# tomerlieber/doc-agents

Hardware: AMD Instinct MI355X
Metric: QA queries/sec + p50 cache-miss latency; docs/min ingest at 1/2/4/8 MI355X (higher is better)
Workload: dtype bf16

## Files before the change

### docagents_amd/models/llama.py

```python
from __future__ import annotations

import numpy as np
import torch

from ..ops import get_ops
from ..ops.reference import interleave_gate_up, rope_table
from .configs import DecoderConfig

EPI_NONE, EPI_SWIGLU, EPI_RESID, EPI_ROPE = 0, 3, 4, 6
_FUSED_ROPE_DECODE = True


class TPContext:

    def __init__(self, rank: int = 0, size: int = 1, group=None, xgmi: bool = True):
        self.rank, self.size, self.group = rank, size, group
        self.use_xgmi = xgmi
        self.xgmi = None
        self.xgmi_norm = None

    def setup_device(self, device: torch.device) -> None:
        if self.size > 1 and device.type == "cuda" and self.xgmi is None and self.use_xgmi:
            from ..parallel.xgmi_allreduce import XgmiAllReduce
            self.xgmi = XgmiAllReduce.create(self.group, device)
            if self.xgmi is not None:
                self.xgmi_norm = XgmiAllReduce.create(self.group, device, max_bytes=512 << 10)

    def close(self) -> None:
        comms = [c for c in (self.xgmi, self.xgmi_norm) if c is not None]
        if not comms:
            return
        import torch.distributed as dist
        dist.barrier(group=self.group)
# ... 202 lines not shown
    def _attn_out_and_mlp(self, L, a, x):
        o, tp = self.ops, self.tp
        if tp.size == 1 or tp.rank == 0:
            self._gemm1(L, "wo", a, epi=EPI_RESID, resid=x, out=x)
        else:
            o.gemm(a, L["wo"], out=x)
        tp.all_reduce_(x)
        return self._mlp(L, x)

    def _mlp(self, L, x):
        o, tp = self.ops, self.tp
        if o.gemv_fusable(x.shape[0], L["w_gu"].shape[0], x.shape[1], EPI_SWIGLU):
            g = self._gemm1(L, "w_gu", x, epi=EPI_SWIGLU, rms=(self._gain(L["ln_mlp"]), self.cfg.eps))
        else:
            h = o.rmsnorm(x, L["ln_mlp"], self.cfg.eps)
            g = o.gemm(h, L["w_gu"], epi=EPI_SWIGLU)
        if tp.size == 1 or tp.rank == 0:
            self._gemm1(L, "w_down", g, epi=EPI_RESID, resid=x, out=x)
        else:
            o.gemm(g, L["w_down"], out=x)
        tp.all_reduce_(x)
        return x

    def _logits(self, hlast, gather: bool = True, out=None):
        o = self.ops
        if o.gemv_fusable(hlast.shape[0], self.w["lm_head"].shape[0], hlast.shape[1]):
            logits = self._gemm1(self.w, "lm_head", hlast.contiguous(), rms=(self._gain(self.w["norm"]), self.cfg.eps),
                                 out=None if gather else out)
        else:
            h = o.rmsnorm(hlast, self.w["norm"], self.cfg.eps)
            logits = o.gemm(h, self.w["lm_head"], out=None if gather else out)
        return self.tp.all_gather_cols(logits) if gather else logits

    def sample(self, logits, temperature: float, seed: int, step: int = 0, **kw):
        return tp_sample(self.ops, self.tp, logits, temperature, seed, step, **kw)

    def prefill(self, ids: torch.Tensor, pos: torch.Tensor, slot_tok: torch.Tensor, cu: torch.Tensor,
                max_seqlen: int, last_idx: torch.Tensor, prefix: tuple[int, int] | None = None,
                local_logits: bool = False) -> torch.Tensor:
        c, o, cache = self.cfg, self.ops, self.cache
        D, hl, kl = c.head_dim, self.hl, self.kl
        x = o.embed(ids, self.w["embed"])
        hook = self.layer_hook
        kv_from_cache = bool(getattr(o, "flash_kv_cache_ok", lambda *_: False)(D, True))
        for li, L in enumerate(self.w["layers"]):
            if hook is not None:
                hook(li)
            h = o.rmsnorm(x, L["ln_attn"], c.eps)
            qkv = o.gemm_rope(h, L["wqkv"], pos, self.cos_sin, hl, kl, D, slot_tok, cache.k(li), cache.v(li),
                              kv_out=not kv_from_cache)
            pre = None if prefix is None else (cache.k(li)[prefix[0]], cache.v(li)[prefix[0]], prefix[1])
            if kv_from_cache:
                a = o.flash_attn_varlen(qkv[:, :hl * D], None, None, cu, max_seqlen, hl, kl, D, causal=True,
                                        prefix=pre, kv_cache=(cache.k(li), cache.v(li), slot_tok, pos))
            else:
                a = o.flash_attn_varlen(qkv[:, :hl * D], qkv[:, hl * D:(hl + kl) * D], qkv[:, (hl + kl) * D:], cu,
                                        max_seqlen, hl, kl, D, causal=True, prefix=pre)
            del qkv, h
            x = self._attn_out_and_mlp(L, a, x)
        return self._logits(x.index_select(0, last_idx), gather=not local_logits)

    def decode_step(self, st: "DecodeState") -> torch.Tensor:
        c, o, cache = self.cfg, self.ops, self.cache
        D, hl, kl = c.head_dim, self.hl, self.kl
        x = o.embed(st.tokens, self.w["embed"], out=st.x)
        if self._dk_decode(x.shape[0]):
            return self._decode_step_dk(st, x)
        if self._norm_fusable(x.shape[0]):
            return self._decode_step_fused_norms(st, x)
        if self.tp.size > 1 and x.shape[0] > 1:
            return self._decode_step_tp_fused_norms(st, x)
        fuse = o.gemv_fusable(x.shape[0], self.w["layers"][0]["wqkv"].shape[0], x.shape[1])
        for li, L in enumerate(self.w["layers"]):
            if fuse:
                qkv = self._gemm1(L, "wqkv", x, out=st.qkv, rms=(self._gain(L["ln_attn"]), c.eps))
            else:
                h = o.rmsnorm(x, L["ln_attn"], c.eps, out=st.h)
                qkv = o.gemm(h, L["wqkv"], out=st.qkv)
            a = self._decode_attn(qkv, li, st)
            self._attn_out_and_mlp(L, a, x)
        logits = self._logits(x, gather=False, out=st.logits)
# ... 140 lines not shown
```

### docagents_amd/ops/csrc/attention.hip

```cpp
#include "common.h"

#include <cstdlib>

#pragma clang fp contract(on)

template <int D, int NW = 4, int QH = 1>
struct FA2Cfg {
  static constexpr int KT = 64, QW = 32 * QH, QB = QW * NW, NT = 64 * NW;
  static constexpr int KSTR = D * 2 + 16;
  static constexpr int VSTR = (D == 64) ? 192 : (D == 128) ? 320 : D * 2;
  static constexpr int KBUF = KT * KSTR, VBUF = KT * VSTR;
  static constexpr int CPR = D / 8, LPT = (KT * CPR + NT - 1) / NT;
  static constexpr int SMEM = 2 * (KBUF + VBUF);
};

struct FaPrefix {
  const bf16_t* k;
  const bf16_t* v;
  long long hstride;
  int len;
  int rev;
  const int* kv_slot;
  const int* kv_pos;
  const bf16_t* kc;
  const bf16_t* vc;
  long long slot_stride;
};

struct FaBlock {
  int qb, h, b;
};
__device__ __forceinline__ FaBlock fa_block(int rev, int causal, int G) {
  const int X = gridDim.x, Y = gridDim.y, Z = gridDim.z;
  const bool lpt = causal && (rev & 1);
  if ((rev & 2) && G >= 1 && Y % G == 0 && ((Y / G) * Z) % 8 == 0) {
    const int g = blockIdx.x + X * (blockIdx.y + Y * blockIdx.z);
    const int xcd = g & 7, s = g >> 3;
    const int per = X * G;
    const int pair = (s / per) * 8 + xcd, r = s % per;
    const int qi = r / G, gh = r % G;
    const int hkv = Y / G;
    return FaBlock{lpt ? X - 1 - qi : qi, (pair % hkv) * G + gh, pair / hkv};
  }
  return FaBlock{lpt ? X - 1 - (int)blockIdx.x : (int)blockIdx.x, (int)blockIdx.y, (int)blockIdx.z};
}

template <int D, int NW, int QH, typename T = BF16T>
__global__ void __launch_bounds__(64 * NW, QH == 1 ? 8 / NW : 1)
flash_attn_v2_kernel(const bf16_t* __restrict__ q, const bf16_t* __restrict__ k, const bf16_t* __restrict__ v,
                     int ldq, int ldk, int ldv, const int* __restrict__ cu, int H, int Hkv, int causal,
                     float c, bf16_t* __restrict__ o, int ldo, FaPrefix pre) {
  using C = FA2Cfg<D, NW, QH>;
  constexpr int KT = C::KT, NDS = D / 16, NDB = D / 32, CPR = C::CPR, LPT = C::LPT, NT = C::NT;
  constexpr bool EVEN = (KT * CPR) % NT == 0;
  extern __shared__ __attribute__((aligned(16))) char smem[];

  const FaBlock fb = fa_block(pre.rev, causal, H / Hkv);
  const int b = fb.b, h = fb.h, qb = fb.qb;
  const int s0 = cu[b], L = cu[b + 1] - s0;
  const int q0 = qb * C::QB;
  if (q0 >= L) return;
  const int hk = h / (H / Hkv);
  const int tid = threadIdx.x, lane = tid & 63, wid = tid >> 6;
  const int qr = lane & 31, hi = lane >> 5;
  const int wq0 = q0 + wid * C::QW;
  int qi[QH];
  bool qvalid[QH];
  bf16x8_t qf[QH][NDS];
  f32x16_t oacc[QH][NDB];
  float m_run[QH], l_part[QH];
#pragma unroll
  for (int j = 0; j < QH; ++j) {
    qi[j] = wq0 + 32 * j + qr;
    qvalid[j] = qi[j] < L;
#pragma unroll
    for (int ds = 0; ds < NDS; ++ds) {
      if (qvalid[j]) qf[j][ds] = *(const bf16x8_t*)(q + (size_t)(s0 + qi[j]) * ldq + h * D + ds * 16 + hi * 8);
      else qf[j][ds] = bf16x8_t{0, 0, 0, 0, 0, 0, 0, 0};
    }
#pragma unroll
    for (int i = 0; i < NDB; ++i)
#pragma unroll
// ... 221 lines not shown
      "s_add_u32 m0, m0, 0x400\n\t"
      "s_nop 0\n\t"
      "buffer_load_dwordx4 %3, %4, %6 offen lds\n\t"
      "s_mov_b32 m0, %0"
      : "=&s"(keep)
      : "v"(v0), "v"(v1), "v"(v2), "s"(rs), "s"(lds), "s"(soff)
      : "memory", "scc");
}

template <int D, bool SPEC, bool DMA>
__global__ void __launch_bounds__(256, 2)
flash_attn_pipe_kernel(const bf16_t* __restrict__ q, const bf16_t* __restrict__ k, const bf16_t* __restrict__ v,
                       int ldq, int ldk, int ldv, const int* __restrict__ cu, int H, int Hkv, int causal,
                       float c, bf16_t* __restrict__ o, int ldo, FaPrefix pre) {
  using C = FA2Cfg<D, 4, 1>;
  constexpr int KT = C::KT, NDS = D / 16, NDB = D / 32, CPR = C::CPR, LPT = C::LPT, NT = C::NT;
  constexpr bool EVEN = (KT * CPR) % NT == 0;
  static_assert(NDS <= 6, "pipelined flash: D <= 96");
  static_assert(!DMA || (D == 96 && C::VSTR == D * 2), "DMA tiles: D = 96 (linear V rows)");
  constexpr int KSTR = DMA ? D * 2 : C::KSTR, KBUF = KT * KSTR, TBUF = KBUF + C::VBUF;
  extern __shared__ __attribute__((aligned(16))) char smem[];

  const FaBlock fb = fa_block(pre.rev, causal, H / Hkv);
  const int b = fb.b, h = fb.h, qb = fb.qb;
  const int s0 = cu[b], L = cu[b + 1] - s0;
  const int q0 = qb * C::QB;
  if (q0 >= L) return;
  const int hk = h / (H / Hkv);
  const int tid = threadIdx.x, lane = tid & 63, wid = tid >> 6;
  const int qr = lane & 31, hi = lane >> 5;
  const int wq0 = q0 + wid * C::QW;
  const int qi = wq0 + qr;
  const bool qvalid = qi < L;
  bf16x8_t qf[NDS];
#pragma unroll
  for (int ds = 0; ds < NDS; ++ds)
    qf[ds] = qvalid ? *(const bf16x8_t*)(q + (size_t)(s0 + qi) * ldq + h * D + ds * 16 + hi * 8)
                    : bf16x8_t{0, 0, 0, 0, 0, 0, 0, 0};
  f32x16_t oacc[NDB];
#pragma unroll
  for (int i = 0; i < NDB; ++i)
#pragma unroll
    for (int r = 0; r < 16; ++r) oacc[i][r] = 0.f;
  float m_run = -INFINITY, l_part = 0.f;

  const int P = pre.len, Lk = P + L;
  const int kv_end = causal ? min(Lk, P + q0 + C::QB) : Lk;
  const int wave_end = causal ? min(Lk, P + wq0 + C::QW) : Lk;
// ... 1207 lines not shown
#define FA_ARGS16 (const bf16_t*)q, (const bf16_t*)k, (const bf16_t*)v, ldq, ldk, ldv, (const int*)cu_seqlens, H, Hkv, \
                  causal, scale * 1.4426950408889634f, (bf16_t*)o, ldo, pre
  switch (D) {
    case 64: flash_attn_v2_kernel<64, 4, 1, F16T><<<grid, 256, FA2Cfg<64, 4, 1>::SMEM, s>>>(FA_ARGS16); break;
    case 96: flash_attn_v2_kernel<96, 4, 1, F16T><<<grid, 256, FA2Cfg<96, 4, 1>::SMEM, s>>>(FA_ARGS16); break;
    default: return (int)hipErrorInvalidValue;
  }
#undef FA_ARGS16
  return (int)hipGetLastError();
}

template <int NW, int QH>
static int launch_fa2(const void* q, const void* k, const void* v, int ldq, int ldk, int ldv, const void* cu_seqlens,
                      int B, int max_seqlen, int H, int Hkv, int D, int causal, float sl2e, void* o, int ldo,
                      FaPrefix pre, hipStream_t s) {
  static bool attr_set = false;
  if constexpr (NW * QH <= 8) {
    if (!attr_set) {
      (void)hipFuncSetAttribute((const void*)flash_attn_v2_kernel<128, NW, QH>, hipFuncAttributeMaxDynamicSharedMemorySize,
                                FA2Cfg<128, NW, QH>::SMEM);
      attr_set = true;
    }
  }
  dim3 grid((max_seqlen + 32 * QH * NW - 1) / (32 * QH * NW), H, B);
#define FA_ARGS (const bf16_t*)q, (const bf16_t*)k, (const bf16_t*)v, ldq, ldk, ldv, (const int*)cu_seqlens, H, Hkv, \
                causal, sl2e, (bf16_t*)o, ldo, pre
  switch (D) {
    case 32: flash_attn_v2_kernel<32, NW, QH><<<grid, 64 * NW, FA2Cfg<32, NW, QH>::SMEM, s>>>(FA_ARGS); break;
    case 64: flash_attn_v2_kernel<64, NW, QH><<<grid, 64 * NW, FA2Cfg<64, NW, QH>::SMEM, s>>>(FA_ARGS); break;
    case 96:
      if constexpr (NW * QH <= 8) flash_attn_v2_kernel<96, NW, QH><<<grid, 64 * NW, FA2Cfg<96, NW, QH>::SMEM, s>>>(FA_ARGS);
      else return (int)hipErrorInvalidValue;
      break;
    case 128:
      if constexpr (NW * QH <= 8) flash_attn_v2_kernel<128, NW, QH><<<grid, 64 * NW, FA2Cfg<128, NW, QH>::SMEM, s>>>(FA_ARGS);
      else return (int)hipErrorInvalidValue;
      break;
    default: return (int)hipErrorInvalidValue;
  }
#undef FA_ARGS
  return (int)hipGetLastError();
}

template <int D, bool DMA>
static constexpr int fa_pipe_smem() {
  return 3 * ((DMA ? 64 * D * 2 : FA2Cfg<D, 4, 1>::KBUF) + FA2Cfg<D, 4, 1>::VBUF);
}

template <bool DMA>
static int launch_fa_pipe(const void* q, const void* k, const void* v, int ldq, int ldk, int ldv, const void* cu_seqlens,
                          int B, int max_seqlen, int H, int Hkv, int causal, float sl2e, void* o, int ldo,
                          FaPrefix pre, hipStream_t s) {
  static bool attr_set = false;
  if (!attr_set) {
    (void)hipFuncSetAttribute((const void*)flash_attn_pipe_kernel<96, true, DMA>,
                              hipFuncAttributeMaxDynamicSharedMemorySize, fa_pipe_smem<96, DMA>());
    attr_set = true;
  }
  dim3 grid((max_seqlen + 127) / 128, H, B);
  flash_attn_pipe_kernel<96, true, DMA><<<grid, 256, fa_pipe_smem<96, DMA>(), s>>>(
      (const bf16_t*)q, (const bf16_t*)k, (const bf16_t*)v, ldq, ldk, ldv, (const int*)cu_seqlens, H, Hkv, causal, sl2e,
      (bf16_t*)o, ldo, pre);
  return (int)hipGetLastError();
}

DA_EXPORT int da_flash_attn_v2(const void* q, const void* k, const void* v, int ldq, int ldk, int ldv,
                               const void* cu_seqlens, int B, int max_seqlen, int H, int Hkv, int D, int causal,
                               float scale, void* o, int ldo, const void* pre_k, const void* pre_v,
                               long long pre_hstride, int pre_len, const void* kv_slot, const void* kv_pos,
                               const void* k_cache, const void* v_cache, void* stream) {
  const bool from_cache = kv_slot != nullptr;
  if (from_cache) {
    if (!causal || D != 96 || !kv_pos || !k_cache || !v_cache || pre_hstride < (long long)D ||
        pre_hstride % D || ((uintptr_t)k_cache | (uintptr_t)v_cache) % 16)
      return (int)hipErrorInvalidValue;
    k = k_cache; v = v_cache; ldk = ldv = D;
  }
  if (H % Hkv || ldq % 8 || ldk % 8 || ldv % 8 || ldo % 4) return (int)hipErrorInvalidValue;
  if (pre_len < 0 || (pre_len > 0 && (!pre_k || !pre_v || pre_hstride < (long long)pre_len * D)))
    return (int)hipErrorInvalidValue;
  if (B == 0 || max_seqlen == 0) return 0;
  const float sl2e = scale * 1.4426950408889634f;
  hipStream_t s = (hipStream_t)stream;
  const FaPrefix pre{(const bf16_t*)pre_k, (const bf16_t*)pre_v, pre_hstride, pre_len, kFaDispatch,
                     (const int*)kv_slot, (const int*)kv_pos, (const bf16_t*)k_cache, (const bf16_t*)v_cache,
                     from_cache ? (long long)Hkv * pre_hstride : 0LL};
  if (causal && D == 96) {
    const bool dma = pre_len % 64 == 0 && ((uintptr_t)k | (uintptr_t)v | (uintptr_t)pre_k | (uintptr_t)pre_v) % 16 == 0;
    if (dma) return launch_fa_pipe<true>(q, k, v, ldq, ldk, ldv, cu_seqlens, B, max_seqlen, H, Hkv, causal, sl2e, o, ldo, pre, s);
    return launch_fa_pipe<false>(q, k, v, ldq, ldk, ldv, cu_seqlens, B, max_seqlen, H, Hkv, causal, sl2e, o, ldo, pre, s);
  }
  if (D == 128) return launch_fa2<8, 1>(q, k, v, ldq, ldk, ldv, cu_seqlens, B, max_seqlen, H, Hkv, D, causal, sl2e, o, ldo, pre, s);
  return launch_fa2<4, 1>(q, k, v, ldq, ldk, ldv, cu_seqlens, B, max_seqlen, H, Hkv, D, causal, sl2e, o, ldo, pre, s);
}
```

### docagents_amd/ops/csrc/gemm.hip

```cpp
#include "gemm.h"

template <int BM, int BN, int WM, int WN, int EPI, int PF = 1>
__global__ void __launch_bounds__(256)
gemm_bf16_kernel(GemmArgs p) {
  constexpr int BK = 64;
  constexpr int TM = BM / WM, TN = BN / WN;
  constexpr int FM = TM / 16, FN = TN / 16;
  constexpr int A_BYTES = BM * BK * 2, B_BYTES = BN * BK * 2;
  constexpr int LA = BM * 8 / 256, LB = BN * 8 / 256;
  static_assert(WM * WN == 4, "4 waves");
  static_assert(LA >= 1 && LB >= 1, "tile too small");
  constexpr int STAGE_FLOATS = 4 * TM * (TN + 4);
  constexpr int LDS_MAIN = 2 * (A_BYTES + B_BYTES);
  constexpr int LDS_BYTES = LDS_MAIN > STAGE_FLOATS * 4 ? LDS_MAIN : STAGE_FLOATS * 4;
  __shared__ __attribute__((aligned(16))) char smem[LDS_BYTES];

  const int tid = threadIdx.x, lane = tid & 63, wid = tid >> 6;
  const int wm = wid / WN, wn = wid % WN;

  const int ntm = (p.M + BM - 1) / BM, ntn = (p.N + BN - 1) / BN;
  const int nwg = ntm * ntn;
  const int t = xcd_remap(blockIdx.x, nwg);
  constexpr int GROUP = 8;
  const int gid = t / (GROUP * ntn);
// ... 507 lines not shown
  const int nout = (epi == EPI_SWIGLU) ? N / 2 : N;
  const size_t work = (size_t)M * (nout / 8);
  const int blocks = (int)((work + 255) / 256);
  gemm_splitk_reduce<<<blocks, 256, 0, s>>>((const float*)ws, splits, M, N, epi, (const bf16_t*)bias,
                                             (const bf16_t*)resid, ldr, (bf16_t*)C, ldc, ssq_in, ssq_parts, norm_k,
                                             eps);
  DA_LAUNCH_CHECK();
}

DA_EXPORT int da_gemm_rope(const void* A, int lda, const void* W, void* C, int ldc, int M, int N, int K,
                           const void* pos, const void* slot, const void* cos_sin, void* k_cache, void* v_cache,
                           int H, int Hkv, int D, int max_seq, int kv_out, void* stream) {
  if (K % 64 || K < 128 || N % 8 || lda % 8 || ldc % 8 || D % 8 || M < 256) return (int)hipErrorInvalidValue;
  if (N != (H + 2 * Hkv) * D || !pos || !slot || !cos_sin || !k_cache || !v_cache) return (int)hipErrorInvalidValue;
  GemmArgs a{};
  a.A = (const bf16_t*)A; a.W = (const bf16_t*)W; a.C = (bf16_t*)C;
  a.M = M; a.N = N; a.K = K; a.lda = lda; a.ldc = ldc; a.k_per_split = K;
  a.rope = RopeArgs{(const int*)pos, (const int*)slot, (const float*)cos_sin, (bf16_t*)k_cache, (bf16_t*)v_cache,
                    H, Hkv, D, max_seq, kv_out ? 1 : 0};
  const long t256 = (long)((M + 255) / 256) * ((N + 255) / 256);
  return launch_gemm8p(a, EPI_ROPE, (hipStream_t)stream, t256 >= 256 ? 256 : 128);
}

DA_EXPORT int da_gemm_bf16(const void* A, int lda, const void* W, void* C, int ldc,
                           const void* bias, const void* resid, int ldr,
                           int M, int N, int K, int epi, int tile, int splits, void* ws,
                           const void* rms_gamma, float rms_eps, void* stream) {
  hipStream_t s = (hipStream_t)stream;
  if (K % 64 || N % 8 || lda % 8 || ldc % 8) return (int)hipErrorInvalidValue;
  if (epi == EPI_SWIGLU && N % 32) return (int)hipErrorInvalidValue;
  if (splits < 1) splits = 1;
  if ((K / 64) % splits) return (int)hipErrorInvalidValue;
  if (splits > 1 && ws == nullptr) return (int)hipErrorInvalidValue;
  GemmArgs a{};
  a.A = (const bf16_t*)A; a.W = (const bf16_t*)W; a.C = (bf16_t*)C;
  a.bias = (const bf16_t*)bias; a.resid = (const bf16_t*)resid; a.ws = (float*)ws;
  a.M = M; a.N = N; a.K = K; a.lda = lda; a.ldc = ldc; a.ldr = ldr; a.k_per_split = K / splits;
  a.gamma = (const bf16_t*)rms_gamma; a.eps = rms_eps;
  if ((rms_gamma || rms_eps > 0.f) && tile != 6) return (int)hipErrorInvalidValue;
  if (tile == 0) {
    if (M <= 32) tile = 3;
    else if (M < 640 || splits > 1) tile = 2;
    else if (K < 128) tile = 1;
    else tile = gemm8p_pick_bm(M, N) == 256 ? 7 : 10;
  }
  if (tile == 4 || tile == 7 || tile == 10) {
    if (splits != 1 || K < 128) return (int)hipErrorInvalidValue;
    return launch_gemm8p(a, epi, s, tile == 10 ? 128 : 256);
  }
  if (tile == 13) {
    if (splits != 1 || K < 128) return (int)hipErrorInvalidValue;
    return launch_gemm4w(a, epi, s);
  }
  if (tile == 6) return launch_gemv(a, epi, s);
  int err;
  switch (tile) {
    case 1: err = launch_tile<128, 128, 2, 2>(a, epi, splits, s); break;
    case 2: err = launch_decode_tile<64, 128>(a, epi, splits, s); break;
    case 3: err = launch_decode_tile<32, 128>(a, epi, splits, s); break;
    case 8: err = launch_tile<128, 128, 2, 2, 4>(a, epi, splits, s); break;
    case 9: err = launch_tile<128, 64, 2, 2, 4>(a, epi, splits, s); break;
    default: return (int)hipErrorInvalidValue;
  }
  if (err || splits == 1) return err;
  const int nout = (epi == EPI_SWIGLU) ? N / 2 : N;
  const size_t work = (size_t)M * (nout / 8);
  int blocks = (int)((work + 255) / 256);
  if (blocks > 4096) blocks = 4096;
// ... 5 lines not shown
```

### docagents_amd/ops/csrc/norm.hip

```cpp
#include "common.h"

#define MAXCH 8

template <typename T = BF16T>
__device__ __forceinline__ void load8(const bf16_t* p, float* v) {
  u32x4_t u = *(const u32x4_t*)p;
#pragma unroll
  for (int e = 0; e < 4; ++e) {
    v[2 * e] = T::to_f((bf16_t)(u[e] & 0xffff));
    v[2 * e + 1] = T::to_f((bf16_t)(u[e] >> 16));
  }
}
template <typename T = BF16T>
__device__ __forceinline__ void store8(bf16_t* p, const float* v) {
  *(u32x4_t*)p = u32x4_t{T::pack2(v[0], v[1]), T::pack2(v[2], v[3]), T::pack2(v[4], v[5]), T::pack2(v[6], v[7])};
}

__global__ void rmsnorm_kernel(const bf16_t* __restrict__ x, bf16_t* __restrict__ resid,
                               const bf16_t* __restrict__ w, bf16_t* __restrict__ y, int D, float eps,
                               int ldx, int ldy) {
  __shared__ float red[16];
  const int row = blockIdx.x;
  const bf16_t* xr = x + (size_t)row * ldx;
  bf16_t* rr = resid ? resid + (size_t)row * D : nullptr;
// ... 294 lines not shown
  if (threadIdx.x == 0) scale[row] = sc;
#pragma unroll
  for (int i = 0; i < MAXCH; ++i) {
    const int c = threadIdx.x + i * blockDim.x;
    if (c < nch) {
      int lo = __builtin_amdgcn_cvt_pk_fp8_f32(v[i][0] * inv, v[i][1] * inv, 0, false);
      lo = __builtin_amdgcn_cvt_pk_fp8_f32(v[i][2] * inv, v[i][3] * inv, lo, true);
      int hi = __builtin_amdgcn_cvt_pk_fp8_f32(v[i][4] * inv, v[i][5] * inv, 0, false);
      hi = __builtin_amdgcn_cvt_pk_fp8_f32(v[i][6] * inv, v[i][7] * inv, hi, true);
      *(u32x2_t*)(out + (size_t)row * ldo + c * 8) = u32x2_t{(unsigned)lo, (unsigned)hi};
    }
  }
}

static inline int row_threads(int D) {
  int ch = D / 8;
  int t = ((ch + 63) / 64) * 64;
  if (t > 256) t = 256;
  if (t < 64) t = 64;
  return t;
}
static inline bool d_ok(int D) { return D % 8 == 0 && D / 8 <= MAXCH * 256; }

DA_EXPORT int da_rmsnorm(const void* x, int ldx, void* resid, const void* w, void* y, int ldy, int M, int D,
                         float eps, void* stream) {
  if (!d_ok(D) || ldx % 8 || ldy % 8) return (int)hipErrorInvalidValue;
  if (M == 0) return 0;
  if (M >= 1024 && D % 512 == 0 && D / 512 <= 8) {
    const dim3 grid((M + 3) / 4);
#define RMS_ROWS(N) rmsnorm_rows_kernel<N><<<grid, 256, 0, (hipStream_t)stream>>>((const bf16_t*)x, (bf16_t*)resid, \
                      (const bf16_t*)w, (bf16_t*)y, M, D, eps, ldx, ldy)
    switch (D / 512) {
      case 4: RMS_ROWS(4); break;
      case 6: RMS_ROWS(6); break;
      case 8: RMS_ROWS(8); break;
      default: rmsnorm_kernel<<<M, row_threads(D), 0, (hipStream_t)stream>>>((const bf16_t*)x, (bf16_t*)resid,
                                                                           (const bf16_t*)w, (bf16_t*)y, D, eps,
                                                                           ldx, ldy);
    }
#undef RMS_ROWS
    DA_LAUNCH_CHECK();
  }
  rmsnorm_kernel<<<M, row_threads(D), 0, (hipStream_t)stream>>>((const bf16_t*)x, (bf16_t*)resid,
                                                                 (const bf16_t*)w, (bf16_t*)y, D, eps, ldx, ldy);
  DA_LAUNCH_CHECK();
}

DA_EXPORT int da_layernorm(const void* x, const void* resid, const void* g, const void* b, void* y, int M, int D,
                           float eps, void* stream) {
  if (!d_ok(D)) return (int)hipErrorInvalidValue;
  if (M == 0) return 0;
  layernorm_kernel<<<M, row_threads(D), 0, (hipStream_t)stream>>>((const bf16_t*)x, (const bf16_t*)resid,
                                                                   (const bf16_t*)g, (const bf16_t*)b,
                                                                   (bf16_t*)y, D, eps);
  DA_LAUNCH_CHECK();
}

DA_EXPORT int da_bert_embed_ln(const void* ids, const void* positions, const void* types, const void* word,
                               const void* pos, const void* type, const void* g, const void* b, void* y, int T,
                               int D, float eps, void* stream) {
  if (!d_ok(D)) return (int)hipErrorInvalidValue;
  if (T == 0) return 0;
  bert_embed_ln_kernel<<<T, row_threads(D), 0, (hipStream_t)stream>>>(
      (const int*)ids, (const int*)positions, (const int*)types, (const bf16_t*)word, (const bf16_t*)pos,
      (const bf16_t*)type, (const bf16_t*)g, (const bf16_t*)b, (bf16_t*)y, D, eps);
  DA_LAUNCH_CHECK();
}

// ... 109 lines not shown
```

### docagents_amd/ops/kernels.py

```python
from __future__ import annotations

import contextlib
import ctypes
import math
import os
import threading
from pathlib import Path

import torch

_LIB = None
_LOCK = threading.Lock()
_DEBUG = os.environ.get("DA_KERNELS_DEBUG", "0") == "1"
_LIB_PATH = Path(__file__).resolve().parent / ("_da_kernels_debug.so" if _DEBUG else "_da_kernels.so")

EPI_NONE, EPI_BIAS, EPI_GELU, EPI_SWIGLU, EPI_RESID = 0, 1, 2, 3, 4
EPI_ROPE = 6

c_longlong = ctypes.c_longlong
c_void_p, c_int, c_float, c_uint, c_size_t = (ctypes.c_void_p, ctypes.c_int, ctypes.c_float,
                                             ctypes.c_uint, ctypes.c_size_t)

_SIGS = {
    "da_gemm_bf16": [c_void_p, c_int, c_void_p, c_void_p, c_int, c_void_p, c_void_p, c_int,
                     c_int, c_int, c_int, c_int, c_int, c_int, c_void_p, c_void_p, c_float, c_void_p],
    "da_gemm_rope": [c_void_p, c_int, c_void_p, c_void_p, c_int, c_int, c_int, c_int] + [c_void_p] * 5
                    + [c_int] * 5 + [c_void_p],
    "da_gemm_fp8": [c_void_p, c_int, c_void_p, c_void_p, c_void_p, c_void_p, c_int, c_void_p, c_void_p, c_int,
                    c_int, c_int, c_int, c_int, c_void_p],
    "da_gemv_w8": [c_void_p, c_void_p, c_void_p, c_void_p, c_void_p, c_void_p, c_int, c_int, c_int, c_void_p, c_float,
                   c_void_p],
    "da_quant_fp8_rows": [c_void_p, c_int, c_int, c_int, c_void_p, c_int, c_void_p, c_void_p],
    "da_layernorm_q": [c_void_p] * 7 + [c_int, c_int, c_float, c_void_p],
    "da_bert_embed_ln_q": [c_void_p] * 11 + [c_int, c_int, c_float, c_void_p],
    "da_gemm_resid_rmsnorm": [c_void_p, c_int, c_void_p, c_void_p, c_int, c_void_p, c_void_p, c_int, c_int, c_int,
                              c_int, c_int, c_int, c_void_p, c_void_p, c_float, c_void_p, c_int, c_void_p],
    "da_rmsnorm": [c_void_p, c_int, c_void_p, c_void_p, c_void_p, c_int, c_int, c_int, c_float, c_void_p],
    "da_swiglu_interleaved": [c_void_p, c_int, c_void_p, c_int, c_int, c_int, c_void_p],
    "da_layernorm": [c_void_p, c_void_p, c_void_p, c_void_p, c_void_p, c_int, c_int, c_float, c_void_p],
    "da_bert_embed_ln": [c_void_p] * 9 + [c_int, c_int, c_float, c_void_p],
    "da_embed": [c_void_p, c_void_p, c_void_p, c_int, c_int, c_void_p],
    "da_pool_l2norm": [c_void_p, c_void_p, c_int, c_int, c_int, c_void_p, c_void_p, c_void_p],
    "da_rope_cache": [c_void_p] * 6 + [c_int] * 6 + [c_void_p],
    "da_sample": [c_void_p, c_int, c_int, c_int, c_float, c_uint, c_uint] + [c_void_p] * 9
                 + [c_int] * 5 + [c_void_p],
    "da_flash_attn_v2": [c_void_p, c_void_p, c_void_p, c_int, c_int, c_int, c_void_p, c_int, c_int,
                         c_int, c_int, c_int, c_int, c_float, c_void_p, c_int, c_void_p, c_void_p, c_longlong,
                         c_int, c_void_p, c_void_p, c_void_p, c_void_p, c_void_p],
    "da_malloc_uncached": [c_longlong, ctypes.POINTER(c_void_p)],
    "da_gemm_dk": [c_void_p, c_int, c_void_p, c_void_p, c_int, c_void_p, c_void_p, c_int, c_int, c_int, c_int,
                   c_int, c_void_p, c_int, c_int, c_float, c_void_p, c_void_p],
    "da_gemm_dk_parts": [c_int],
    "da_gemm_dk_splitk": [c_void_p, c_int, c_void_p, c_void_p, c_int, c_void_p, c_void_p, c_int, c_int, c_int, c_int,
                          c_int, c_void_p, c_int, c_int, c_float, c_void_p, c_void_p, c_int, c_void_p],
    "da_decode_attn": [c_void_p, c_int, c_void_p, c_void_p, c_void_p, c_void_p, c_void_p, c_int, c_int, c_int, c_int,
                       c_int, c_int, c_int, c_float, c_void_p, c_void_p, c_int, c_void_p, c_void_p, c_void_p,
                       c_int, c_void_p],
    "da_topk_dense": [c_void_p, c_int, c_int, c_void_p, c_void_p, c_int, c_void_p, c_int, c_float, c_int,
                      c_int, c_void_p, c_void_p, c_void_p, c_void_p],
    "da_topk_dense_stream": [c_void_p, c_int, c_int, c_void_p, c_void_p, c_int, c_void_p, c_int, c_float, c_int,
                             c_int, c_void_p, c_void_p, c_void_p, c_void_p],
    "da_topk_ranges": [c_void_p, c_int, c_void_p, c_void_p, c_int, c_void_p, c_void_p, c_void_p, c_int,
                       c_float, c_int, c_int, c_int, c_void_p, c_void_p, c_void_p, c_void_p],
    "da_topk_merge": [c_void_p, c_void_p, c_int, c_int, c_int, c_void_p, c_void_p, c_void_p],
    "da_kmeans_accum": [c_void_p, c_int, c_int, c_void_p, c_void_p, c_void_p, c_void_p],
    "da_sample_partial": [c_void_p, c_int, c_int, c_int, c_int, c_float, c_uint, c_uint, c_void_p, c_void_p, c_void_p],
    "da_sample_chunked": [c_void_p, c_int, c_int, c_int, c_float, c_uint, c_uint] + [c_void_p] * 10
                         + [c_int] * 5 + [c_void_p],
    "da_sample_finalize": [c_void_p, c_int, c_int] + [c_void_p] * 8 + [c_int] * 5 + [c_void_p],
    "da_stream_create_cumask": [c_uint, ctypes.POINTER(c_uint), ctypes.POINTER(c_void_p)],
    "da_stream_get_cumask": [c_void_p, c_uint, ctypes.POINTER(c_uint)],
# ... 148 lines not shown
    if (tile == 12 or (tile == 0 and splits <= 0)) and rms is None and dk_fusable(M, N, K, epi):
        return gemm_dk(a, w, epi=epi, bias=bias, resid=resid, out=out)
    if tile == 0 and splits <= 0 and gemv_fusable(M, N, K, epi):
        tile, splits = 6, 1
    gamma, eps = (None, 0.0) if rms is None else rms
    if rms is not None:
        _req(tile == 6, "fused RMSNorm needs the M == 1 GEMV path")
        _req(eps > 0, "fused RMSNorm needs eps > 0")
        if gamma is not None:
            _bf16_cuda(gamma, "gamma"); _req(gamma.numel() == K, "gamma must be [K]")
    if splits <= 0:
        if tile == 0 and M < 640:
            tile = _decode_tile(M, N)
        splits = _auto_splits(M, N, K) if tile in (0, 2, 3) or (tile == 9 and M <= 128) else 1
    ws = None
    if splits > 1:
        ws = _workspace(splits * M * N * 4, a.device)
    rc = lib().da_gemm_bf16(_ptr(a), a.stride(0), _ptr(w), _ptr(out), out.stride(0), _ptr(bias), _ptr(resid), ldr,
                            M, N, K, epi, tile, splits, _ptr(ws), _ptr(gamma), float(eps), _stream())
    _check(rc, "gemm")
    return out


DECODE_DK = True
DK_MAX_M = 64
DK_SPLITK_ABOVE = 32


def dk_fusable(M: int, N: int, K: int, epi: int = EPI_NONE) -> bool:
    return (DECODE_DK and 2 <= M <= DK_MAX_M and K % 256 == 0 and N % 16 == 0
            and epi in (EPI_NONE, EPI_BIAS, EPI_RESID, EPI_SWIGLU) and (epi != EPI_SWIGLU or N % 32 == 0))


def _dk_splitk(M: int, N: int) -> bool:
    return DK_SPLITK_ABOVE < M <= 64 and N % 512 == 0


def _dk_splits(N: int, K: int) -> int:
    tiles, ks = (N + 127) // 128, K // 64
    best = 2
    for s in (2, 3, 4, 6, 8, 12, 16):
        if ks % s == 0 and ks // s >= 4 and tiles * s <= 256:
            best = s
    return best if ks % best == 0 else 2


# ... 196 lines not shown
        return 2 if N >= 8192 else 9
    return 2


def _auto_splits(M: int, N: int, K: int) -> int:
    if M >= 640:
        return 1
    ksteps = K // 64
    if 64 < M <= 128:
        if N >= 8192:
            return 1
        s = 4
        while s > 1 and (ksteps % s or ksteps // s < 4):
            s //= 2
        return s
    tiles = math.ceil(M / (32 if _decode_tile(M) == 3 else 64)) * math.ceil(N / 128)
    cap = 256 if M <= 64 else (1024 if M < 256 else 640)
    s = 1
    while tiles * s * 2 <= cap and ksteps % (s * 2) == 0 and ksteps // (s * 2) >= 4:
        s *= 2
    return s


def rmsnorm(x, w, eps: float, resid=None, out=None):
    _bf16_cuda(x, "x"); _bf16_cuda(w, "w")
    M, D = x.shape
    _req(x.stride(1) == 1 and x.stride(0) % 8 == 0 and D % 8 == 0, "x must be row-major, D % 8 == 0")
    _req(w.numel() == D, "w must be [D]")
    if resid is not None:
        _bf16_cuda(resid, "resid"); _req(resid.is_contiguous() and resid.shape == (M, D), "resid must be [M, D]")
    if out is None:
        out = torch.empty((M, D), dtype=torch.bfloat16, device=x.device)
    _req(out.stride(1) == 1 and out.stride(0) % 8 == 0, "bad out")
    _check(lib().da_rmsnorm(_ptr(x), x.stride(0), _ptr(resid), _ptr(w), _ptr(out), out.stride(0), M, D,
                            float(eps), _stream()), "rmsnorm")
    return out


def layernorm(x, g, b, eps: float, resid=None, out=None, fp8_out: bool = False):
    _bf16_cuda(x, "x")
    M, D = x.shape
    _req(x.is_contiguous() and D % 8 == 0, "x must be contiguous, D % 8 == 0")
    if resid is not None:
        _req(resid.is_contiguous() and resid.shape == x.shape, "bad resid")
    if out is None:
        out = torch.empty_like(x)
    if fp8_out:
        yq = torch.empty((M, D), dtype=FP8, device=x.device)
        ys = torch.empty(M, dtype=torch.float32, device=x.device)
        _check(lib().da_layernorm_q(_ptr(x), _ptr(resid), _ptr(g), _ptr(b), _ptr(out), _ptr(yq), _ptr(ys), M, D,
                                    float(eps), _stream()), "layernorm_q")
        return out, yq, ys
    _check(lib().da_layernorm(_ptr(x), _ptr(resid), _ptr(g), _ptr(b), _ptr(out), M, D, float(eps), _stream()),
           "layernorm")
    return out


def bert_embed_ln(ids, positions, types, word, pos, type_, g, b, eps: float, out=None, fp8_out: bool = False):
# ... 40 lines not shown

def rope_cache(qkv, pos, cos_sin, H, Hkv, D, slot=None, k_cache=None, v_cache=None, rotate_q=True):
    _bf16_cuda(qkv, "qkv"); _i32(pos, "pos")
    T = qkv.shape[0]
    _req(qkv.is_contiguous() and qkv.shape[1] == (H + 2 * Hkv) * D, "qkv shape")
    _req(cos_sin.dtype == torch.float32 and cos_sin.is_contiguous() and cos_sin.shape[-1] == 2
         and cos_sin.shape[1] == D // 2, "cos_sin must be fp32 [max_pos, D/2, 2]")
    max_seq = 0
    if k_cache is not None:
        _i32(slot, "slot")
        _req(k_cache.is_contiguous() and v_cache.is_contiguous() and k_cache.shape == v_cache.shape, "caches")
        _req(k_cache.dim() == 4 and k_cache.shape[1] == Hkv and k_cache.shape[3] == D, "cache [S, Hkv, max_seq, D]")
        max_seq = k_cache.shape[2]
    _check(lib().da_rope_cache(_ptr(qkv), _ptr(pos), _ptr(slot), _ptr(cos_sin), _ptr(k_cache), _ptr(v_cache),
                               T, H, Hkv, D, max_seq, 1 if rotate_q else 0, _stream()), "rope_cache")
    return qkv


def flash_kv_cache_ok(D: int, causal: bool) -> bool:
    return causal and D == 96


def flash_attn_varlen(q, k, v, cu_seqlens, max_seqlen: int, H: int, Hkv: int, D: int, causal: bool,
                      scale: float | None = None, out=None, prefix=None, kv_cache=None):
    kc = vc = ks = kpos = None
    if kv_cache is not None:
        kc, vc, ks, kpos = kv_cache
        _req(flash_kv_cache_ok(D, causal), "kv_cache: causal D = 96 only")
        _bf16_cuda(kc, "k_cache"); _bf16_cuda(vc, "v_cache"); _i32(ks, "slot"); _i32(kpos, "pos")
        _req(kc.is_contiguous() and vc.is_contiguous() and kc.shape == vc.shape and kc.dim() == 4
             and kc.shape[1] == Hkv and kc.shape[3] == D, "caches [slots, Hkv, max_seq, D]")
        _req(ks.numel() >= q.shape[0] and kpos.numel() >= q.shape[0], "slot / pos per token")
        k = v = q
    for t, n in ((q, "q"), (k, "k"), (v, "v")):
        _bf16_cuda(t, n)
        _req(t.dim() == 2 and t.stride(1) == 1 and t.stride(0) % 8 == 0 and t.data_ptr() % 16 == 0, f"{n} layout")
    _i32(cu_seqlens, "cu_seqlens")
    _req(D in (32, 64, 96, 128), f"head dim {D} unsupported")
    _req(H % Hkv == 0, "H % Hkv")
    T = q.shape[0]
    if out is None:
        out = torch.empty((T, H * D), dtype=torch.bfloat16, device=q.device)
    scale = scale if scale is not None else 1.0 / math.sqrt(D)
    B = cu_seqlens.numel() - 1
    kp = vp = None
    hstride, P = 0, 0
    if prefix is not None:
        kp, vp, P = prefix
        P = int(P)
        _bf16_cuda(kp, "k_pre"); _bf16_cuda(vp, "v_pre")
        _req(kp.dim() == 3 and kp.shape == vp.shape and kp.shape[0] == Hkv and kp.shape[2] == D
             and kp.is_contiguous() and vp.is_contiguous() and 0 <= P <= kp.shape[1], "prefix K/V [Hkv, max_seq, D]")
        hstride = kp.shape[1] * D
    if kc is not None:
        _req(prefix is None or kp.shape[1] == kc.shape[2], "prefix and caches differ in max_seq")
        hstride = kc.shape[2] * D
    _check(lib().da_flash_attn_v2(_ptr(q), _ptr(k), _ptr(v), q.stride(0), k.stride(0), v.stride(0),
                                  _ptr(cu_seqlens), B, int(max_seqlen), H, Hkv, D, int(causal), float(scale),
                                  _ptr(out), out.stride(0), _ptr(kp), _ptr(vp), hstride, P, _ptr(ks), _ptr(kpos),
                                  _ptr(kc), _ptr(vc), _stream()),
           "flash_attn_varlen")
    return out


_FUSED_COMBINE = True
_UC: dict = {}


class _RawBuf:

    def __init__(self, ptr: int, nbytes: int):
        self.ptr, self.nbytes = ptr, nbytes

    def data_ptr(self) -> int:
        return self.ptr


def _uncached(tag: str, nbytes: int, device) -> _RawBuf:
    key = (tag, device.index if device.index is not None else torch.cuda.current_device(),
           getattr(_ROLE, "name", "main"))
    bufs = _UC.setdefault(key, [])
    if not bufs or bufs[-1].nbytes < nbytes:
        n = max(nbytes, 1 << 20)
# ... 363 lines not shown
```

### docagents_amd/ops/reference.py

```python
from __future__ import annotations

import math

import numpy as np
import torch
import torch.nn.functional as F

EPI_NONE, EPI_BIAS, EPI_GELU, EPI_SWIGLU, EPI_RESID = 0, 1, 2, 3, 4
EPI_ROPE = 6


def gemv_fusable(M, N, K, epi=EPI_NONE):
    return M == 1


def gemm(a, w, bias=None, epi=EPI_NONE, resid=None, out=None, rms=None, **_):
    if rms is not None:
        g = rms[0] if rms[0] is not None else torch.ones(a.shape[1], dtype=a.dtype, device=a.device)
        a = rmsnorm(a, g, rms[1])
    return _epilogue(a.float() @ w.float().t(), w.shape[0], bias, epi, resid, out)


def _epilogue(y, N, bias, epi, resid, out):
    if bias is not None:
        y = y + bias.float()
    if epi == EPI_GELU:
        y = F.gelu(y)
    elif epi == EPI_SWIGLU:
        yy = y.view(y.shape[0], N // 32, 2, 16)
        g, u = yy[:, :, 0, :], yy[:, :, 1, :]
        y = (F.silu(g) * u).reshape(y.shape[0], N // 2)
    elif epi == EPI_RESID:
        y = y + resid.float()
    y = y.to(torch.bfloat16)
    if out is not None:
        out.copy_(y)
# ... 4 lines not shown
def gemm_f16(a, w, bias=None, epi=EPI_NONE, resid=None, out=None):
    y = a.float() @ w.float().t()
    if bias is not None:
        y = y + bias.float()
    if epi == EPI_GELU:
        y = F.gelu(y)
    elif epi == EPI_RESID:
        y = y + resid.float()
    y = y.to(torch.float16)
    if out is not None:
        out.copy_(y)
        return out
    return y


def interleave_gate_up(gate: torch.Tensor, up: torch.Tensor) -> torch.Tensor:
    Fd, K = gate.shape
    assert Fd % 16 == 0
    g = gate.view(Fd // 16, 16, K)
    u = up.view(Fd // 16, 16, K)
    return torch.stack([g, u], dim=1).reshape(2 * Fd, K).contiguous()


def rmsnorm(x, w, eps, resid=None, out=None):
    xf = x.float()
    if resid is not None:
        xf = xf + resid.float()
        resid.copy_(xf.to(resid.dtype))
    y = xf * torch.rsqrt(xf.pow(2).mean(-1, keepdim=True) + eps) * w.float()
    y = y.to(x.dtype)
    if out is not None:
        out.copy_(y)
        return out
    return y


def layernorm(x, g, b, eps, resid=None, out=None, fp8_out=False):
    xf = x.float()
    if resid is not None:
        xf = xf + resid.float()
    yf = F.layer_norm(xf, (xf.shape[-1],), g.float(), None if b is None else b.float(), eps)
    y = yf.to(x.dtype)
    if out is not None:
        out.copy_(y)
        y = out
    if fp8_out:
        yq, ys = quant_fp8(yf)
# ... 52 lines not shown
    qkv = gemm(a, w, out=out)
    return rope_cache(qkv, pos, cos_sin, H, Hkv, D, slot=slot, k_cache=k_cache, v_cache=v_cache)


def rope_cache(qkv, pos, cos_sin, H, Hkv, D, slot=None, k_cache=None, v_cache=None, rotate_q=True):
    T = qkv.shape[0]
    x = qkv.view(T, H + 2 * Hkv, D)
    cs = cos_sin[pos.long()]
    if rotate_q:
        x[:, :H] = _rope_rows(x[:, :H], cs).to(qkv.dtype)
    x[:, H:H + Hkv] = _rope_rows(x[:, H:H + Hkv], cs).to(qkv.dtype)
    if k_cache is not None:
        sl, ps = slot.long(), pos.long()
        k_cache[sl, :, ps] = x[:, H:H + Hkv]
        v_cache[sl, :, ps] = x[:, H + Hkv:]
    return qkv


def flash_kv_cache_ok(D: int, causal: bool) -> bool:
    return causal


def flash_attn_varlen(q, k, v, cu_seqlens, max_seqlen, H, Hkv, D, causal, scale=None, out=None, prefix=None,
                      kv_cache=None):
    if kv_cache is not None:
        kc, vc, ks, kpos = kv_cache
        T = q.shape[0]
        cu = cu_seqlens.tolist()
        k = torch.empty((T, Hkv * D), dtype=q.dtype, device=q.device)
        v = torch.empty((T, Hkv * D), dtype=q.dtype, device=q.device)
        for b in range(len(cu) - 1):
            s0, s1 = cu[b], cu[b + 1]
            if s1 > s0:
                sl, p0 = int(ks[s0]), int(kpos[s0])
                k[s0:s1] = kc[sl, :, p0:p0 + s1 - s0].transpose(0, 1).reshape(s1 - s0, Hkv * D)
                v[s0:s1] = vc[sl, :, p0:p0 + s1 - s0].transpose(0, 1).reshape(s1 - s0, Hkv * D)
    scale = scale if scale is not None else 1.0 / math.sqrt(D)
    T = q.shape[0]
    res = torch.empty((T, H * D), dtype=q.dtype, device=q.device)
    cu = cu_seqlens.tolist()
    G = H // Hkv
    P = 0 if prefix is None else int(prefix[2])
    if P:
        kp = prefix[0][:, :P].float().repeat_interleave(G, 0)
        vp = prefix[1][:, :P].float().repeat_interleave(G, 0)
    for b in range(len(cu) - 1):
        s0, s1 = cu[b], cu[b + 1]
        L = s1 - s0
        if L == 0:
            continue
        qq = q[s0:s1, :H * D].float().view(L, H, D).transpose(0, 1)
        kk = k[s0:s1, :Hkv * D].float().view(L, Hkv, D).transpose(0, 1).repeat_interleave(G, 0)
        vv = v[s0:s1, :Hkv * D].float().view(L, Hkv, D).transpose(0, 1).repeat_interleave(G, 0)
        if P:
            kk, vv = torch.cat([kp, kk], 1), torch.cat([vp, vv], 1)
        s = (qq @ kk.transpose(1, 2)) * scale
        if causal:
            m = torch.ones(L, P + L, dtype=torch.bool, device=q.device).triu(P + 1)
            s = s.masked_fill(m, float("-inf"))
        p = s.softmax(-1)
        res[s0:s1] = (p @ vv).transpose(0, 1).reshape(L, H * D).to(q.dtype)
    if out is not None:
        out.copy_(res)
        return out
    return res


def decode_attn(q, k_cache, v_cache, lens, slot, H, Hkv, D, max_len=None, chunk=256, scale=None, out=None, pre=None,
                rope=None):
    if rope is not None:
        q = rope_cache(q.clone(), rope[1], rope[0], H, Hkv, D, slot=slot, k_cache=k_cache, v_cache=v_cache)
    scale = scale if scale is not None else 1.0 / math.sqrt(D)
    B = q.shape[0]
    G = H // Hkv
    res = torch.empty((B, H * D), dtype=q.dtype, device=q.device)
    pre_h = None if pre is None else pre.tolist()
    for b in range(B):
        L, s = int(lens[b]), int(slot[b])
        qq = q[b, :H * D].float().view(H, 1, D)
        kk = k_cache[s, :, :L].float()
        vv = v_cache[s, :, :L].float()
        if pre_h is not None and pre_h[b][0] > 0:
            P, ps = pre_h[b]
            kk = torch.cat([k_cache[ps, :, :P].float(), kk[:, P:]], 1)
# ... 301 lines not shown
```

Before: 35.49.

## Compute only last-token rows in final prefill layer attention and MLP

In the last decoder layer during prefill, attention runs only the final query block of each sequence, and the output projection, MLP and norm run only on the rows needed for logits (last_idx). GEMM tile and split routes and the rmsnorm kernel choice are pinned to the full-M values so numerics match the full path. This removes most of the last layer's attention and MLP work in prefill. The risk is that it relies on last_idx pointing to the final token of each sequence. It also adds plumbing: a new kernel arg, a route export and an env toggle.

```diff
diff --git a/docagents_amd/models/llama.py b/docagents_amd/models/llama.py
--- a/docagents_amd/models/llama.py
+++ b/docagents_amd/models/llama.py
@@ -1,4 +1,6 @@
 from __future__ import annotations
+
+import os
 
 import numpy as np
 import torch
@@ -9,6 +11,7 @@
 
 EPI_NONE, EPI_SWIGLU, EPI_RESID, EPI_ROPE = 0, 3, 4, 6
 _FUSED_ROPE_DECODE = True
+_PREFILL_TAIL = os.environ.get("DA_PREFILL_TAIL", "1") != "0"
 
 
 class TPContext:
@@ -257,6 +260,27 @@
         tp.all_reduce_(x)
         return x
 
+    def _tail_routes(self, M: int):
+        if not _PREFILL_TAIL:
+            return None
+        L = self.w["layers"][-1]
+        prods = (("wo", EPI_RESID), ("w_gu", EPI_SWIGLU), ("w_down", EPI_RESID))
+        routes = [self.ops.gemm_route(M, L[k].shape[0], L[k].shape[1], e) for k, e in prods]
+        return None if any(r is None for r in routes) else routes
+
+    def _attn_out_and_mlp_rows(self, L, a, x, routes, M: int):
+        o, tp = self.ops, self.tp
+        first = tp.size == 1 or tp.rank == 0
+        res = dict(epi=EPI_RESID, resid=x) if first else {}
+        r_o, r_gu, r_down = routes
+        o.gemm(a, L["wo"], out=x, **res, **r_o)
+        tp.all_reduce_(x)
+        h = o.rmsnorm(x, L["ln_mlp"], self.cfg.eps, route_m=M)
+        g = o.gemm(h, L["w_gu"], epi=EPI_SWIGLU, **r_gu)
+        o.gemm(g, L["w_down"], out=x, **res, **r_down)
+        tp.all_reduce_(x)
+        return x
+
     def _logits(self, hlast, gather: bool = True, out=None):
         o = self.ops
         if o.gemv_fusable(hlast.shape[0], self.w["lm_head"].shape[0], hlast.shape[1]):
@@ -278,6 +302,8 @@
         x = o.embed(ids, self.w["embed"])
         hook = self.layer_hook
         kv_from_cache = bool(getattr(o, "flash_kv_cache_ok", lambda *_: False)(D, True))
+        M, last = x.shape[0], len(self.w["layers"]) - 1
+        tail = self._tail_routes(M)
         for li, L in enumerate(self.w["layers"]):
             if hook is not None:
                 hook(li)
@@ -285,13 +311,18 @@
             qkv = o.gemm_rope(h, L["wqkv"], pos, self.cos_sin, hl, kl, D, slot_tok, cache.k(li), cache.v(li),
                               kv_out=not kv_from_cache)
             pre = None if prefix is None else (cache.k(li)[prefix[0]], cache.v(li)[prefix[0]], prefix[1])
+            cut = tail is not None and li == last
             if kv_from_cache:
                 a = o.flash_attn_varlen(qkv[:, :hl * D], None, None, cu, max_seqlen, hl, kl, D, causal=True,
-                                        prefix=pre, kv_cache=(cache.k(li), cache.v(li), slot_tok, pos))
+                                        prefix=pre, kv_cache=(cache.k(li), cache.v(li), slot_tok, pos),
+                                        tail_only=cut)
             else:
                 a = o.flash_attn_varlen(qkv[:, :hl * D], qkv[:, hl * D:(hl + kl) * D], qkv[:, (hl + kl) * D:], cu,
-                                        max_seqlen, hl, kl, D, causal=True, prefix=pre)
+                                        max_seqlen, hl, kl, D, causal=True, prefix=pre, tail_only=cut)
             del qkv, h
+            if cut:
+                x = self._attn_out_and_mlp_rows(L, a.index_select(0, last_idx), x.index_select(0, last_idx), tail, M)
+                return self._logits(x, gather=not local_logits)
             x = self._attn_out_and_mlp(L, a, x)
         return self._logits(x.index_select(0, last_idx), gather=not local_logits)
 
diff --git a/docagents_amd/ops/csrc/attention.hip b/docagents_amd/ops/csrc/attention.hip
--- a/docagents_amd/ops/csrc/attention.hip
+++ b/docagents_amd/ops/csrc/attention.hip
@@ -25,6 +25,7 @@
   const bf16_t* kc;
   const bf16_t* vc;
   long long slot_stride;
+  int tail;
 };
 
 struct FaBlock {
@@ -45,6 +46,10 @@
   return FaBlock{lpt ? X - 1 - (int)blockIdx.x : (int)blockIdx.x, (int)blockIdx.y, (int)blockIdx.z};
 }
 
+__device__ __forceinline__ int fa_query_block(const FaBlock& fb, int tail, int L, int QB) {
+  return tail ? (L > 0 ? (L - 1) / QB : 0) : fb.qb;
+}
+
 template <int D, int NW, int QH, typename T = BF16T>
 __global__ void __launch_bounds__(64 * NW, QH == 1 ? 8 / NW : 1)
 flash_attn_v2_kernel(const bf16_t* __restrict__ q, const bf16_t* __restrict__ k, const bf16_t* __restrict__ v,
@@ -56,8 +61,9 @@
   extern __shared__ __attribute__((aligned(16))) char smem[];
 
   const FaBlock fb = fa_block(pre.rev, causal, H / Hkv);
-  const int b = fb.b, h = fb.h, qb = fb.qb;
+  const int b = fb.b, h = fb.h;
   const int s0 = cu[b], L = cu[b + 1] - s0;
+  const int qb = fa_query_block(fb, pre.tail, L, C::QB);
   const int q0 = qb * C::QB;
   if (q0 >= L) return;
   const int hk = h / (H / Hkv);
@@ -325,8 +331,9 @@
   extern __shared__ __attribute__((aligned(16))) char smem[];
 
   const FaBlock fb = fa_block(pre.rev, causal, H / Hkv);
-  const int b = fb.b, h = fb.h, qb = fb.qb;
+  const int b = fb.b, h = fb.h;
   const int s0 = cu[b], L = cu[b + 1] - s0;
+  const int qb = fa_query_block(fb, pre.tail, L, C::QB);
   const int q0 = qb * C::QB;
   if (q0 >= L) return;
   const int hk = h / (H / Hkv);
@@ -1580,7 +1587,7 @@
       attr_set = true;
     }
   }
-  dim3 grid((max_seqlen + 32 * QH * NW - 1) / (32 * QH * NW), H, B);
+  dim3 grid(pre.tail ? 1 : (max_seqlen + 32 * QH * NW - 1) / (32 * QH * NW), H, B);
 #define FA_ARGS (const bf16_t*)q, (const bf16_t*)k, (const bf16_t*)v, ldq, ldk, ldv, (const int*)cu_seqlens, H, Hkv, \
                 causal, sl2e, (bf16_t*)o, ldo, pre
   switch (D) {
@@ -1615,7 +1622,7 @@
                               hipFuncAttributeMaxDynamicSharedMemorySize, fa_pipe_smem<96, DMA>());
     attr_set = true;
   }
-  dim3 grid((max_seqlen + 127) / 128, H, B);
+  dim3 grid(pre.tail ? 1 : (max_seqlen + 127) / 128, H, B);
   flash_attn_pipe_kernel<96, true, DMA><<<grid, 256, fa_pipe_smem<96, DMA>(), s>>>(
       (const bf16_t*)q, (const bf16_t*)k, (const bf16_t*)v, ldq, ldk, ldv, (const int*)cu_seqlens, H, Hkv, causal, sl2e,
       (bf16_t*)o, ldo, pre);
@@ -1626,7 +1633,7 @@
                                const void* cu_seqlens, int B, int max_seqlen, int H, int Hkv, int D, int causal,
                                float scale, void* o, int ldo, const void* pre_k, const void* pre_v,
                                long long pre_hstride, int pre_len, const void* kv_slot, const void* kv_pos,
-                               const void* k_cache, const void* v_cache, void* stream) {
+                               const void* k_cache, const void* v_cache, int tail_only, void* stream) {
   const bool from_cache = kv_slot != nullptr;
   if (from_cache) {
     if (!causal || D != 96 || !kv_pos || !k_cache || !v_cache || pre_hstride < (long long)D ||
@@ -1642,7 +1649,7 @@
   hipStream_t s = (hipStream_t)stream;
   const FaPrefix pre{(const bf16_t*)pre_k, (const bf16_t*)pre_v, pre_hstride, pre_len, kFaDispatch,
                      (const int*)kv_slot, (const int*)kv_pos, (const bf16_t*)k_cache, (const bf16_t*)v_cache,
-                     from_cache ? (long long)Hkv * pre_hstride : 0LL};
+                     from_cache ? (long long)Hkv * pre_hstride : 0LL, tail_only ? 1 : 0};
   if (causal && D == 96) {
     const bool dma = pre_len % 64 == 0 && ((uintptr_t)k | (uintptr_t)v | (uintptr_t)pre_k | (uintptr_t)pre_v) % 16 == 0;
     if (dma) return launch_fa_pipe<true>(q, k, v, ldq, ldk, ldv, cu_seqlens, B, max_seqlen, H, Hkv, causal, sl2e, o, ldo, pre, s);
diff --git a/docagents_amd/ops/csrc/gemm.hip b/docagents_amd/ops/csrc/gemm.hip
--- a/docagents_amd/ops/csrc/gemm.hip
+++ b/docagents_amd/ops/csrc/gemm.hip
@@ -553,6 +553,17 @@
   return launch_gemm8p(a, EPI_ROPE, (hipStream_t)stream, t256 >= 256 ? 256 : 128);
 }
 
+static int auto_tile(int M, int N, int K, int splits) {
+  if (M <= 32) return 3;
+  if (M < 640 || splits > 1) return 2;
+  if (K < 128) return 1;
+  return gemm8p_pick_bm(M, N) == 256 ? 7 : 10;
+}
+
+DA_EXPORT int da_gemm_route(int M, int N, int K, int splits) {
+  return auto_tile(M, N, K, splits < 1 ? 1 : splits);
+}
+
 DA_EXPORT int da_gemm_bf16(const void* A, int lda, const void* W, void* C, int ldc,
                            const void* bias, const void* resid, int ldr,
                            int M, int N, int K, int epi, int tile, int splits, void* ws,
@@ -569,12 +580,7 @@
   a.M = M; a.N = N; a.K = K; a.lda = lda; a.ldc = ldc; a.ldr = ldr; a.k_per_split = K / splits;
   a.gamma = (const bf16_t*)rms_gamma; a.eps = rms_eps;
   if ((rms_gamma || rms_eps > 0.f) && tile != 6) return (int)hipErrorInvalidValue;
-  if (tile == 0) {
-    if (M <= 32) tile = 3;
-    else if (M < 640 || splits > 1) tile = 2;
-    else if (K < 128) tile = 1;
-    else tile = gemm8p_pick_bm(M, N) == 256 ? 7 : 10;
-  }
+  if (tile == 0) tile = auto_tile(M, N, K, splits);
   if (tile == 4 || tile == 7 || tile == 10) {
     if (splits != 1 || K < 128) return (int)hipErrorInvalidValue;
     return launch_gemm8p(a, epi, s, tile == 10 ? 128 : 256);
diff --git a/docagents_amd/ops/csrc/norm.hip b/docagents_amd/ops/csrc/norm.hip
--- a/docagents_amd/ops/csrc/norm.hip
+++ b/docagents_amd/ops/csrc/norm.hip
@@ -340,11 +340,11 @@
 }
 static inline bool d_ok(int D) { return D % 8 == 0 && D / 8 <= MAXCH * 256; }
 
-DA_EXPORT int da_rmsnorm(const void* x, int ldx, void* resid, const void* w, void* y, int ldy, int M, int D,
-                         float eps, void* stream) {
+static int rmsnorm_launch(const void* x, int ldx, void* resid, const void* w, void* y, int ldy, int M, int D,
+                          float eps, int route_m, void* stream) {
   if (!d_ok(D) || ldx % 8 || ldy % 8) return (int)hipErrorInvalidValue;
   if (M == 0) return 0;
-  if (M >= 1024 && D % 512 == 0 && D / 512 <= 8) {
+  if (route_m >= 1024 && D % 512 == 0 && D / 512 <= 8) {
     const dim3 grid((M + 3) / 4);
 #define RMS_ROWS(N) rmsnorm_rows_kernel<N><<<grid, 256, 0, (hipStream_t)stream>>>((const bf16_t*)x, (bf16_t*)resid, \
                       (const bf16_t*)w, (bf16_t*)y, M, D, eps, ldx, ldy)
@@ -362,6 +362,16 @@
   rmsnorm_kernel<<<M, row_threads(D), 0, (hipStream_t)stream>>>((const bf16_t*)x, (bf16_t*)resid,
                                                                  (const bf16_t*)w, (bf16_t*)y, D, eps, ldx, ldy);
   DA_LAUNCH_CHECK();
+}
+
+DA_EXPORT int da_rmsnorm(const void* x, int ldx, void* resid, const void* w, void* y, int ldy, int M, int D,
+                         float eps, void* stream) {
+  return rmsnorm_launch(x, ldx, resid, w, y, ldy, M, D, eps, M, stream);
+}
+
+DA_EXPORT int da_rmsnorm_routed(const void* x, int ldx, void* resid, const void* w, void* y, int ldy, int M, int D,
+                                float eps, int route_m, void* stream) {
+  return rmsnorm_launch(x, ldx, resid, w, y, ldy, M, D, eps, route_m < M ? M : route_m, stream);
 }
 
 DA_EXPORT int da_layernorm(const void* x, const void* resid, const void* g, const void* b, void* y, int M, int D,
diff --git a/docagents_amd/ops/kernels.py b/docagents_amd/ops/kernels.py
--- a/docagents_amd/ops/kernels.py
+++ b/docagents_amd/ops/kernels.py
@@ -36,6 +36,8 @@
     "da_gemm_resid_rmsnorm": [c_void_p, c_int, c_void_p, c_void_p, c_int, c_void_p, c_void_p, c_int, c_int, c_int,
                               c_int, c_int, c_int, c_void_p, c_void_p, c_float, c_void_p, c_int, c_void_p],
     "da_rmsnorm": [c_void_p, c_int, c_void_p, c_void_p, c_void_p, c_int, c_int, c_int, c_float, c_void_p],
+    "da_rmsnorm_routed": [c_void_p, c_int, c_void_p, c_void_p, c_void_p, c_int, c_int, c_int, c_float, c_int,
+                          c_void_p],
     "da_swiglu_interleaved": [c_void_p, c_int, c_void_p, c_int, c_int, c_int, c_void_p],
     "da_layernorm": [c_void_p, c_void_p, c_void_p, c_void_p, c_void_p, c_int, c_int, c_float, c_void_p],
     "da_bert_embed_ln": [c_void_p] * 9 + [c_int, c_int, c_float, c_void_p],
@@ -46,7 +48,8 @@
                  + [c_int] * 5 + [c_void_p],
     "da_flash_attn_v2": [c_void_p, c_void_p, c_void_p, c_int, c_int, c_int, c_void_p, c_int, c_int,
                          c_int, c_int, c_int, c_int, c_float, c_void_p, c_int, c_void_p, c_void_p, c_longlong,
-                         c_int, c_void_p, c_void_p, c_void_p, c_void_p, c_void_p],
+                         c_int, c_void_p, c_void_p, c_void_p, c_void_p, c_int, c_void_p],
+    "da_gemm_route": [c_int, c_int, c_int, c_int],
     "da_malloc_uncached": [c_longlong, ctypes.POINTER(c_void_p)],
     "da_gemm_dk": [c_void_p, c_int, c_void_p, c_void_p, c_int, c_void_p, c_void_p, c_int, c_int, c_int, c_int,
                    c_int, c_void_p, c_int, c_int, c_float, c_void_p, c_void_p],
@@ -241,6 +244,19 @@
     return out
 
 
+def gemm_route(M: int, N: int, K: int, epi: int = EPI_NONE):
+    if M <= 128:
+        return None
+    if M < 640:
+        tile = _decode_tile(M, N)
+        splits = _auto_splits(M, N, K)
+    else:
+        tile, splits = 0, 1
+    if tile == 0:
+        tile = int(lib().da_gemm_route(M, N, K, splits))
+    return {"tile": tile, "splits": splits}
+
+
 DECODE_DK = True
 DK_MAX_M = 64
 DK_SPLITK_ABOVE = 32
@@ -483,7 +499,7 @@
     return s
 
 
-def rmsnorm(x, w, eps: float, resid=None, out=None):
+def rmsnorm(x, w, eps: float, resid=None, out=None, route_m: int = 0):
     _bf16_cuda(x, "x"); _bf16_cuda(w, "w")
     M, D = x.shape
     _req(x.stride(1) == 1 and x.stride(0) % 8 == 0 and D % 8 == 0, "x must be row-major, D % 8 == 0")
@@ -493,8 +509,8 @@
     if out is None:
         out = torch.empty((M, D), dtype=torch.bfloat16, device=x.device)
     _req(out.stride(1) == 1 and out.stride(0) % 8 == 0, "bad out")
-    _check(lib().da_rmsnorm(_ptr(x), x.stride(0), _ptr(resid), _ptr(w), _ptr(out), out.stride(0), M, D,
-                            float(eps), _stream()), "rmsnorm")
+    _check(lib().da_rmsnorm_routed(_ptr(x), x.stride(0), _ptr(resid), _ptr(w), _ptr(out), out.stride(0), M, D,
+                                   float(eps), int(route_m), _stream()), "rmsnorm")
     return out
 
 
@@ -581,7 +597,7 @@
 
 
 def flash_attn_varlen(q, k, v, cu_seqlens, max_seqlen: int, H: int, Hkv: int, D: int, causal: bool,
-                      scale: float | None = None, out=None, prefix=None, kv_cache=None):
+                      scale: float | None = None, out=None, prefix=None, kv_cache=None, tail_only: bool = False):
     kc = vc = ks = kpos = None
     if kv_cache is not None:
         kc, vc, ks, kpos = kv_cache
@@ -617,7 +633,7 @@
     _check(lib().da_flash_attn_v2(_ptr(q), _ptr(k), _ptr(v), q.stride(0), k.stride(0), v.stride(0),
                                   _ptr(cu_seqlens), B, int(max_seqlen), H, Hkv, D, int(causal), float(scale),
                                   _ptr(out), out.stride(0), _ptr(kp), _ptr(vp), hstride, P, _ptr(ks), _ptr(kpos),
-                                  _ptr(kc), _ptr(vc), _stream()),
+                                  _ptr(kc), _ptr(vc), int(bool(tail_only)), _stream()),
            "flash_attn_varlen")
     return out
 
diff --git a/docagents_amd/ops/reference.py b/docagents_amd/ops/reference.py
--- a/docagents_amd/ops/reference.py
+++ b/docagents_amd/ops/reference.py
@@ -12,6 +12,10 @@
 
 def gemv_fusable(M, N, K, epi=EPI_NONE):
     return M == 1
+
+
+def gemm_route(M, N, K, epi=EPI_NONE):
+    return None if M <= 128 else {}
 
 
 def gemm(a, w, bias=None, epi=EPI_NONE, resid=None, out=None, rms=None, **_):
@@ -62,7 +66,7 @@
     return torch.stack([g, u], dim=1).reshape(2 * Fd, K).contiguous()
 
 
-def rmsnorm(x, w, eps, resid=None, out=None):
+def rmsnorm(x, w, eps, resid=None, out=None, route_m=0):
     xf = x.float()
     if resid is not None:
         xf = xf + resid.float()
@@ -161,7 +165,7 @@
 
 
 def flash_attn_varlen(q, k, v, cu_seqlens, max_seqlen, H, Hkv, D, causal, scale=None, out=None, prefix=None,
-                      kv_cache=None):
+                      kv_cache=None, tail_only=False):
     if kv_cache is not None:
         kc, vc, ks, kpos = kv_cache
         T = q.shape[0]
@@ -199,6 +203,8 @@
             s = s.masked_fill(m, float("-inf"))
         p = s.softmax(-1)
         res[s0:s1] = (p @ vv).transpose(0, 1).reshape(L, H * D).to(q.dtype)
+        if tail_only:
+            res[s0:s0 + (L - 1) // 128 * 128] = float("nan")
     if out is not None:
         out.copy_(res)
         return out
```

After: 35.96, median of 6. 1.01x the previous value.
